# vivian556123/NeurIPS2024-CoVoMix

Hardware: AMD Instinct MI355X
Metric: mel-frames/sec (VoMix 32-step + HiFi-GAN, Bx1000x80) (higher is better)
Workload: dtype f16x3->f32 (fp32 operands split into fp16 hi/lo pairs, 3 MFMA products, fp32 accumulate); 1 GPU; VoMix 32-NFE (16 midpoint steps, CFG 0.7) + HiFi-GAN config_covomix, B=8 utterances x T=1000 frames per GPU, prompt 400; per_gpu_batch=8, frames=1000, nfe=32, parallelism=dp1 (utterance-sharded)

## Files before the change

include/covomix_hip.h:

```cpp
#ifndef COVOMIX_HIP_H
#define COVOMIX_HIP_H

#include <stdint.h>

#ifdef __cplusplus
extern "C" {
#endif

#define CVX_OK      0
#define CVX_EINVAL (-22)
#define CVX_EHIP   (-5)

#define CVX_ACT_NONE 0
#define CVX_ACT_GELU 1
#define CVX_ACT_SILU 2
#define CVX_ACT_TANH 3

typedef struct cvx_ctx {
    void*     stream;
    uint32_t* sat_flag;
    int32_t   n_cus;
    int32_t   flags;
} cvx_ctx;
#define CVX_CTX_NO_SATURATION_FLAG 1
typedef const cvx_ctx* cvx_stream_t;

#define CVX_ABI_VERSION 109
int         cvx_version(void);
const char* cvx_last_error_string(void);

int cvx_saturation_flag_reset(cvx_stream_t ctx);
int cvx_saturation_flag_query(uint32_t* host_out, int32_t reset, cvx_stream_t ctx);

int cvx_clock_stamps(uint64_t* stamps_dev, cvx_stream_t ctx);
int cvx_stream_create_cu_mask(const uint32_t* mask, int32_t n_words, void** out_stream);
int cvx_stream_destroy(void* stream);

typedef struct {
    const float* A;   int64_t lda;
    const float* A2;  int64_t lda2;  int32_t K1;
    const float* W;   int64_t ldw;
    float*       C;   int64_t ldc;
    const float* bias;
    const float* residual; int64_t ldr;
    int32_t M, N, K;
    int32_t act;
    const float* rope_cos; const float* rope_sin; int32_t rope_T; int32_t rope_cols;
} cvx_gemm_args;
int cvx_gemm_bias_act_f32(const cvx_gemm_args* a, cvx_stream_t s);

// ... 53 lines not shown
int cvx_attention_f16x3(const uint16_t* qk_hi, const uint16_t* qk_lo, const uint16_t* vt_hi, const uint16_t* vt_lo,
                        float* out, uint16_t* out_hi, uint16_t* out_lo,
                        int32_t Bt, int32_t T, int32_t Tp, int32_t H, float scale, cvx_stream_t s);
int cvx_attention_f16x3_scaled(const uint16_t* qk_hi, const uint16_t* qk_lo, const uint16_t* vt_hi, const uint16_t* vt_lo,
                               float* out, uint16_t* out_hi, uint16_t* out_lo,
                               int32_t Bt, int32_t T, int32_t Tp, int32_t H, float scale,
                               const float* qk_scale_dev, const float* v_scale_dev, const float* out_scale_dev, cvx_stream_t s);
int cvx_attention_f16x3_varlen(const uint16_t* qk_hi, const uint16_t* qk_lo, const uint16_t* vt_hi, const uint16_t* vt_lo,
                               float* out, uint16_t* out_hi, uint16_t* out_lo, const int32_t* cu_seqlens_dev,
                               int32_t n_seq, int32_t max_T, int64_t M, int32_t vt_ld, int32_t H, float scale,
                               const float* qk_scale_dev, const float* v_scale_dev, const float* out_scale_dev, cvx_stream_t s);

#define CVX_ATT_FORM_A 0
#define CVX_ATT_FORM_B 1
#define CVX_ATT_FORM_C 2
#define CVX_ATT_FORM_SINGLE_TERM 3
int cvx_attention_f16x3_form(int32_t n_seq, int32_t max_T, int64_t q_rows, int32_t H, int32_t single_term,
                             int32_t* query_block, int32_t* key_groups, int32_t* query_waves);

int cvx_dwconv31_gelu_res_f32(const float* x, const float* w, const float* bias, float* y,
                              int32_t Bt, int32_t T, int32_t C, cvx_stream_t s);
int cvx_dwconv31_gelu_res_varlen_f32(const float* x, const float* w, const float* bias, float* y,
                                     const int32_t* cu_seqlens_dev, int32_t n_seq, int32_t max_T, int32_t C, cvx_stream_t s);
int cvx_gemm_skinny_f32(const float* A, int32_t lda, const float* W, int64_t ldw, const float* bias, float* C, int64_t ldc,
                        int32_t M, int32_t N, int32_t K, int32_t act, cvx_stream_t s);
int cvx_cfg_combine_axpy_f32(const float* f_c, const float* f_n, const float* y, float cond_scale,
                             float coef, float* out, float* out2, float* out3, int64_t n, cvx_stream_t s);

int cvx_embed_gather_f32(const int64_t* ids, int32_t S, const float* table, int32_t E, int32_t n_rows_table,
                         const float* cond, const float* cond_row, int32_t Cc, int64_t null_id,
                         float* out, int64_t M, cvx_stream_t s);

int cvx_time_fourier_f32(const float* times, const float* w, float* out, int32_t n, int32_t half,
                         cvx_stream_t s);

typedef struct { const int32_t* item_len_dev; int32_t mul, add; } cvx_item_lengths;
typedef struct {
    const float* x;  int32_t B, Cin, Lin;
    const float* Wp; const float* bias;
    float* out;      int32_t Cout, Lout;
    int32_t ksize, dil, pad, up;
    float in_slope;
    const float* res; const float* accum; float out_scale;
    cvx_item_lengths items;
} cvx_conv_args;
int     cvx_hifigan_conv1d_f32(const cvx_conv_args* a, cvx_stream_t s);
// ... 188 lines not shown
```

neurips2024-covomix_amd/_lib.py:

```python
from __future__ import annotations

import ctypes as C
import os

import torch

_HERE = os.path.dirname(os.path.abspath(__file__))
LIB_PATH = os.environ.get("CVX_LIB_PATH") or os.path.join(_HERE, "libcovomix_hip.so")

_f32p = C.POINTER(C.c_float)
ABI_VERSION = 109


class GemmArgs(C.Structure):
    _fields_ = [
        ("A", C.c_void_p), ("lda", C.c_int64),
        ("A2", C.c_void_p), ("lda2", C.c_int64), ("K1", C.c_int32),
        ("W", C.c_void_p), ("ldw", C.c_int64),
        ("C", C.c_void_p), ("ldc", C.c_int64),
        ("bias", C.c_void_p),
        ("residual", C.c_void_p), ("ldr", C.c_int64),
        ("M", C.c_int32), ("N", C.c_int32), ("K", C.c_int32),
        ("act", C.c_int32),
        ("rope_cos", C.c_void_p), ("rope_sin", C.c_void_p), ("rope_T", C.c_int32), ("rope_cols", C.c_int32),
    ]


class GemmSplitIO(C.Structure):
    _fields_ = [
        ("A_hi", C.c_void_p), ("A_lo", C.c_void_p), ("lda_h", C.c_int64),
        ("A2_hi", C.c_void_p), ("A2_lo", C.c_void_p), ("lda2_h", C.c_int64),
        ("C_hi", C.c_void_p), ("C_lo", C.c_void_p), ("ldc_h", C.c_int64),
        ("write_f32", C.c_int32),
        ("Vt_hi", C.c_void_p), ("Vt_lo", C.c_void_p), ("vt_ld", C.c_int64),
# ... 184 lines not shown
                                                      C.c_int32, C.c_int32, C.c_int32, C.c_float, C.c_void_p, C.c_void_p]),
    "cvx_amax_pow2_scale_f32": (C.c_int, [C.c_void_p, C.c_int64, C.c_float, C.c_void_p, C.c_void_p, C.c_void_p]),
    "cvx_split_f16_dev": (C.c_int, [C.c_void_p, C.c_void_p, C.c_void_p, C.c_int64, C.c_float, C.c_void_p, C.c_void_p]),
    "cvx_split_f16_colscale_il": (C.c_int, [C.c_void_p, C.c_int64, C.c_int32, C.c_int32, C.c_void_p, C.c_int64, C.c_void_p, C.c_int64, C.c_int32,
                                            C.c_float, C.c_void_p, C.c_void_p]),
    "cvx_rownorm_scale_f32": (C.c_int, [C.c_void_p, C.c_int64, C.c_int32, C.c_int64, C.c_float, C.c_float, C.c_void_p, C.c_void_p]),
    "cvx_adarmsnorm_scaled_f32": (C.c_int, [C.c_void_p, C.c_void_p, C.c_void_p, C.c_void_p, C.c_void_p, C.c_void_p, C.c_int64,
                                            C.c_int32, C.c_int64, C.c_float, C.c_float, C.c_void_p, C.c_void_p]),
    "cvx_attention_f16x3_scaled": (C.c_int, [C.c_void_p, C.c_void_p, C.c_void_p, C.c_void_p, C.c_void_p, C.c_void_p, C.c_void_p,
                                             C.c_int32, C.c_int32, C.c_int32, C.c_int32, C.c_float, C.c_void_p, C.c_void_p,
                                             C.c_void_p, C.c_void_p]),
    "cvx_gemm_f16x3": (C.c_int, [C.POINTER(GemmArgs), C.c_void_p, C.c_void_p, C.c_float, C.POINTER(GemmSplitIO),
                                 C.c_void_p]),
    "cvx_gemm_f16x3_norm": (C.c_int, [C.POINTER(GemmArgs), C.c_void_p, C.c_void_p, C.c_float, C.POINTER(GemmSplitIO),
                                      C.POINTER(GemmNorm), C.c_void_p]),
    "cvx_adarmsnorm_f32": (C.c_int, [C.c_void_p, C.c_void_p, C.c_void_p, C.c_void_p, C.c_void_p, C.c_void_p, C.c_int64, C.c_int32,
                                     C.c_int64, C.c_float, C.c_float, C.c_void_p]),
    "cvx_attention_f32": (C.c_int, [C.c_void_p, C.c_void_p, C.c_void_p, C.c_void_p, C.c_int32, C.c_int32, C.c_int32, C.c_float,
                                    C.c_void_p]),
    "cvx_attention_f16x3": (C.c_int, [C.c_void_p, C.c_void_p, C.c_void_p, C.c_void_p, C.c_void_p, C.c_void_p, C.c_void_p,
                                      C.c_int32, C.c_int32, C.c_int32, C.c_int32, C.c_float, C.c_void_p]),
    "cvx_dwconv31_gelu_res_f32": (C.c_int, [C.c_void_p, C.c_void_p, C.c_void_p, C.c_void_p, C.c_int32, C.c_int32,
                                            C.c_int32, C.c_void_p]),
    "cvx_cfg_combine_axpy_f32": (C.c_int, [C.c_void_p, C.c_void_p, C.c_void_p, C.c_float, C.c_float, C.c_void_p,
                                           C.c_void_p, C.c_void_p, C.c_int64, C.c_void_p]),
    "cvx_embed_gather_f32": (C.c_int, [C.c_void_p, C.c_int32, C.c_void_p, C.c_int32, C.c_int32, C.c_void_p,
                                       C.c_void_p, C.c_int32, C.c_int64, C.c_void_p, C.c_int64, C.c_void_p]),
    "cvx_time_fourier_f32": (C.c_int, [C.c_void_p, C.c_void_p, C.c_void_p, C.c_int32, C.c_int32, C.c_void_p]),
    "cvx_hifigan_conv1d_f32": (C.c_int, [C.POINTER(ConvArgs), C.c_void_p]),
    "cvx_hifigan_packed_weight_floats": (C.c_int64, [C.c_int32, C.c_int32, C.c_int32]),
    "cvx_hifigan_pack_weight_f32": (C.c_int, [C.c_void_p, C.c_int32, C.c_int32, C.c_int32, C.c_int32, C.c_void_p]),
    "cvx_hifigan_post_f32": (C.c_int, [C.c_void_p, C.c_void_p, C.c_float, C.c_void_p, C.c_int32, C.c_int32,
                                       C.c_int32, C.c_float, C.c_void_p]),
    "cvx_wav_to_int16": (C.c_int, [C.c_void_p, C.c_void_p, C.c_int64, C.c_void_p]),
    "cvx_saturation_flag_reset": (C.c_int, [C.c_void_p]),
    "cvx_saturation_flag_query": (C.c_int, [C.POINTER(C.c_uint32), C.c_int32, C.c_void_p]),
    "cvx_stream_create_cu_mask": (C.c_int, [C.POINTER(C.c_uint32), C.c_int32, C.POINTER(C.c_void_p)]),
    "cvx_stream_destroy": (C.c_int, [C.c_void_p]),
    "cvx_clock_stamps": (C.c_int, [C.c_void_p, C.c_void_p]),
    "cvx_attention_varlen_f32": (C.c_int, [C.c_void_p, C.c_void_p, C.c_void_p, C.c_void_p, C.c_void_p, C.c_int32, C.c_int32,
                                           C.c_int32, C.c_float, C.c_void_p]),
    "cvx_attention_f16x3_varlen": (C.c_int, [C.c_void_p, C.c_void_p, C.c_void_p, C.c_void_p, C.c_void_p, C.c_void_p, C.c_void_p,
                                             C.c_void_p, C.c_int32, C.c_int32, C.c_int64, C.c_int32, C.c_int32, C.c_float,
                                             C.c_void_p, C.c_void_p, C.c_void_p, C.c_void_p]),
    "cvx_attention_f16x3_form": (C.c_int, [C.c_int32, C.c_int32, C.c_int64, C.c_int32, C.c_int32, C.POINTER(C.c_int32), C.POINTER(C.c_int32),
                                           C.POINTER(C.c_int32)]),
# ... 48 lines not shown
```

neurips2024-covomix_amd/acoustic.py:

```python
from __future__ import annotations

from typing import Dict, List, Optional

import os

import torch

from . import ops


def _dims_from_state(sd: Dict[str, torch.Tensor]) -> dict:
    dim, e_in = sd["to_embed.weight"].shape
    dim_cond = sd["null_cond"].shape[0]
    dim_emb = sd["to_phoneme_emb.weight"].shape[1]
    depth = 0
    while f"transformer.layers.{depth}.2.to_qkv.weight" in sd:
        depth += 1
    inner = sd["transformer.layers.0.2.to_qkv.weight"].shape[0] // 3
    dim_out = sd["to_pred.weight"].shape[0]
    streams = (e_in - dim_out - dim_cond) // dim_emb
    if dim_out + streams * dim_emb + dim_cond != e_in or inner % 64 != 0:
        raise ValueError("unsupported CoVoMix checkpoint geometry")
    return dict(dim=dim, e_in=e_in, dim_cond=dim_cond, dim_emb=dim_emb, depth=depth, heads=inner // 64,
                dim_head=64, dim_out=dim_out, streams=streams,
# ... 290 lines not shown
                and self.d["dim"] % 64 == 0 and 512 <= self.d["dim"] <= 4096 and os.environ.get("CVX_DEFER_NORM", "1") == "1"):
            return False
        return True

    def _deferred_norm_tables(self, table: torch.Tensor, HS: torch.Tensor, times_key) -> dict:
        d, sd = self.d, self.sd
        n, L, dim = table.shape[0], d["depth"], d["dim"]
        tab = table.view(n, L, 4, dim)
        tiny = torch.finfo(torch.float32).tiny
        gmax = tab[:, :, 0::2, :].abs().amax(dim=-1)
        gs = torch.exp2(-torch.ceil(torch.log2(gmax.clamp_min(tiny))).clamp(-40, 40)).contiguous()
        AS = (gs * HS[None, :, 1:3]).contiguous()

        def beta_w(beta_rows: torch.Tensor, w: torch.Tensor, bias) -> torch.Tensor:
            out = torch.empty(n, w.shape[0], dtype=torch.float32, device=self.device)
            for r0 in range(0, n, 32):
                r1 = min(n, r0 + 32)
                ops.gemm_skinny(beta_rows[r0:r1], w, out[r0:r1], bias=bias)
            return out
        key = (n, L, times_key)
        bufs = self._dn_bufs.get(key)
        if bufs is None:
            mk = lambda N: torch.empty(n, N, 2 * dim, dtype=torch.float16, device=self.device)
            bufs = dict(wq=[None if i == 0 else mk(3 * d["heads"] * 64) for i in range(L)], w1=[mk(4 * dim) for _ in range(L)])
            self._dn_bufs[key] = bufs
        b1p, bq, wq, w1 = [], [], [], []
        for i in range(L):
            p = f"transformer.layers.{i}"
            nq, n1 = p + ".2.to_qkv.weight", p + ".4.0.weight"
            b1p.append(beta_w(tab[:, i, 3, :], sd[n1], sd[p + ".4.0.bias"]))
            inv1 = self.split_il[n1][1]
            ops.split_f16_colscale_il(sd[n1], tab[:, i, 2, :], gs[:, i, 1], 1.0 / inv1, bufs["w1"][i])
            w1.append([(bufs["w1"][i][e], inv1) for e in range(n)])
            if i == 0:
                bq.append(None); wq.append(None)
                continue
            bq.append(beta_w(tab[:, i, 1, :], sd[nq], None))
            invq = self.split_il[nq][1]
            ops.split_f16_colscale_il(sd[nq], tab[:, i, 0, :], gs[:, i, 0], 1.0 / invq, bufs["wq"][i])
            wq.append([(bufs["wq"][i][e], invq) for e in range(n)])
        a0, h0 = AS.data_ptr(), HS.data_ptr()
        return dict(b1p=b1p, bq=bq, wq=wq, w1=w1, gs=gs, AS=AS, HS=HS, hsp=[[h0 + 4 * (4 * i + k) for k in range(4)] for i in range(L)],
                         asp=[[(a0 + 4 * ((e * L + i) * 2), a0 + 4 * ((e * L + i) * 2 + 1)) for i in range(L)] for e in range(n)])

    def _layers_pair_stream(self, ctx: dict, step: int, ws: dict, h: torch.Tensor, twin: dict, free: list, Bt: int, T: int, M: int, rg):
        d, sd, dn = self.d, self.sd, ctx["dn"]
        dim, L = d["dim"], d["depth"]
        tab = ctx["table"][step]
        sp, il = self.split.get, self.split_il.get
        sp_step, pp, hsp = ctx["sp"][step], self.pred_scale.data_ptr(), dn["hsp"]
        cur = hsp[0][0]
        take = free.pop
        parts64, rt_dim = dim // 64, float(dim) ** 0.5
        n16, a16, f16 = ws["normed16"], ws["att16"], ws["ff16"]
        rowsq = ws["rowsq"]
        rs = ws["rs"]
        def factor():
            ops.rownorm_scale(rowsq, M, parts64, rs, rt_dim)
        fkw = dict(a_row_scale=rs)
        skips: List[tuple] = []
        have_rs = False
        for i in range(L):
            p = f"transformer.layers.{i}"
            s_na, s_qk, s_v, s_at, s_nf, s_ff = sp_step[i]
            as_a, as_f = dn["asp"][step][i]
            last = i + 1 == L
            if self.has_comb[i]:
                s, s_scale = skips.pop()
                comb = take()
                ops.gemm(h, sd[p + ".0.weight"], comb, bias=sd[p + ".0.bias"], a2=s, w_split=sp(p + ".0.weight"), w_il=il(p + ".0.weight"),
                         a_split=twin[id(h)], a2_split=twin[id(s)], a_scale=cur, a2_scale=s_scale, out_split=twin[id(comb)], c_scale=hsp[i][1],
                         c_rowsq=rowsq, write_f32=False)
                cur = hsp[i][1]
                factor()
                have_rs = True
                free += [h, s]
                h, keep_input = comb, False
            else:
                skips.append((h, cur))
                keep_input = True
            nq = p + ".2.to_qkv.weight"
            if have_rs:
                ops.gemm(ws["normed"], sd[nq], ws["qkv"], rope=ws["rope"], rope_cols=2 * d["heads"] * 64, w_split=sp(nq), w_il=dn["wq"][i][step],
                         a_split=twin[id(h)], out_split=ws["qk16"], vt_split=ws["vt16"], write_f32=False, a_scale=as_a, c_scale=s_qk, vt_scale=s_v,
                         bias=dn["bq"][i][step], **fkw)
            else:
                ops.adarmsnorm(h, tab[(4 * i) * dim:(4 * i + 1) * dim], tab[(4 * i + 1) * dim:(4 * i + 2) * dim], None, out_split=n16, split_scale=s_na)
                ops.gemm(ws["normed"], sd[nq], ws["qkv"], rope=ws["rope"], rope_cols=2 * d["heads"] * 64, w_split=sp(nq), w_il=il(nq),
                         a_split=n16, out_split=ws["qk16"], vt_split=ws["vt16"], write_f32=False, a_scale=s_na, c_scale=s_qk, vt_scale=s_v)
            ops.attention_f16x3(ws["qk16"], ws["vt16"], None, Bt, T, d["heads"], 64 ** -0.5, out_split=a16,
                                qk_scale=s_qk, v_scale=s_v, out_scale=s_at, ragged=rg)
            h_att = take() if keep_input else h
            no = p + ".2.to_out.weight"
            ops.gemm(ws["att"], sd[no], h_att, w_split=sp(no), w_il=il(no), a_split=a16, a_scale=s_at, res_split=twin[id(h)], res_scale=cur,
                     out_split=twin[id(h_att)], c_scale=hsp[i][2], c_rowsq=rowsq, write_f32=False)
            cur = hsp[i][2]
            factor()
            h = h_att
            n1, n2 = p + ".4.0.weight", p + ".4.2.weight"
            ops.gemm(ws["normed"], sd[n1], ws["ff"], bias=dn["b1p"][i][step], act=ops.ACT_GELU, w_split=sp(n1), w_il=dn["w1"][i][step],
                     a_split=twin[id(h)], out_split=f16, write_f32=False, a_scale=as_f, c_scale=s_ff, **fkw)
            next_defers = (not last) and not self.has_comb[i + 1]
            ops.gemm(ws["ff"], sd[n2], h, bias=sd[p + ".4.2.bias"], w_split=sp(n2), w_il=il(n2), a_split=f16, a_scale=s_ff,
                     res_split=twin[id(h)], res_scale=cur, out_split=twin[id(h)], c_scale=hsp[i][3], c_rowsq=rowsq if next_defers else None,
                     write_f32=last)
            cur = hsp[i][3]
            if next_defers:
                factor()
            have_rs = next_defers
        ops.adarmsnorm(h, sd["transformer.final_norm.gamma"], None, None, out_split=ws["pred16"], split_scale=pp)
        ops.gemm(ws["normed"], sd["to_pred.weight"], ws["pred"], w_split=sp("to_pred.weight"), a_split=ws["pred16"], a_scale=pp,
                 w_il=il("to_pred.weight") if isinstance(ws["pred16"], ops.SplitIL) else None)
        return ws["pred"]

    @staticmethod
    def _ws_cut(ws: dict, r0: int, r1: int, vt) -> dict:

        def cut(v, lo=r0, hi=r1):
            if isinstance(v, ops.SplitIL):
                return v.rows_view(lo, hi)
            if isinstance(v, tuple):
                return tuple(None if t is None else t[lo:hi] for t in v)
            if isinstance(v, list):
                return [cut(t, lo, hi) for t in v]
            return v[lo:hi]
        out = {}
        for k, v in ws.items():
            if k == "rope":
                out[k] = v
            elif k == "vt16":
                out[k] = v if vt is None else cut(v, vt[0], vt[1])
            else:
                out[k] = cut(v)
        return out

    def evaluate(self, ctx: dict, step: int) -> torch.Tensor:
        d, sd, ws = self.d, self.sd, ctx["ws"]
        Bt, T, M, rg = ctx["Bt"], ctx["T"], ctx["M"], ctx.get("ragged")
        dim = d["dim"]
        tab = ctx["table"][step]
        free: List[torch.Tensor] = list(ws["h"])
        take = free.pop
        il = self.split_il.get
        if self.precision == "f16":
            split_io = M > 64 and dim % 64 == 0
            sp = self.split.get if split_io else (lambda k: None)
        else:
            split_io = self.precision == "f16x3" and M > 64 and dim % 32 == 0
            sp = self.split.get

        h = take()
        h0 = take()
        ops.gemm(ws["xin"], sd["to_embed.weight"][:, : d["dim_out"]], h0, residual=ws["base"])
        ops.dwconv31_gelu_res(h0, self.dw_w, sd["conv_embed.dw_conv1d.0.bias"], h, Bt, T, ragged=rg)
        free.append(h0)
        twin = {id(b): pr for b, pr in zip(ws["h"], ws["h16"])} if split_io else None
        sp_step = ctx["sp"][step] if (split_io and "sp" in ctx) else None
        hp = ctx["hp"] if sp_step is not None else None
        pp = self.pred_scale.data_ptr() if sp_step is not None else None
        use_dn = split_io and M >= 2048 and ctx.get("dn") is not None
        if split_io:
            tw = twin[id(h)]
            h0s = ctx["dn"]["hsp"][0][0] if use_dn else hp
            ops.split_act_f16(h, tw, scale=h0s) if isinstance(tw, ops.SplitIL) else ops.split_act_f16(h, *tw, scale=h0s)

        fuse_norm = split_io and M < 2048
        normed_ahead = False
        if use_dn:
            return self._layers_pair_stream(ctx, step, ws, h, twin, free, Bt, T, M, rg)
        def tab_rows(i_, k_):
            return tab[(4 * i_ + k_) * dim:(4 * i_ + k_ + 1) * dim]
        skips: List[torch.Tensor] = []
        for i in range(d["depth"]):
            p = f"transformer.layers.{i}"
            g_attn = tab[(4 * i + 0) * dim:(4 * i + 1) * dim]
            b_attn = tab[(4 * i + 1) * dim:(4 * i + 2) * dim]
            g_ff = tab[(4 * i + 2) * dim:(4 * i + 3) * dim]
            b_ff = tab[(4 * i + 3) * dim:(4 * i + 4) * dim]
            if (p + ".0.weight") in sd:
                s = skips.pop()
                comb = take()
                if split_io:
                    nm = dict(gamma=g_attn, beta=b_attn, out_split=ws["normed16"],
                              scale=sp_step[i][0] if sp_step is not None else None) if fuse_norm else None
                    ops.gemm(h, sd[p + ".0.weight"], comb, bias=sd[p + ".0.bias"], a2=s, w_split=sp(p + ".0.weight"), w_il=il(p + ".0.weight"),
                             a_split=twin[id(h)], a2_split=twin[id(s)], a_scale=hp, norm=nm)
                    normed_ahead = nm is not None
                else:
                    ops.gemm(h, sd[p + ".0.weight"], comb, bias=sd[p + ".0.bias"], a2=s, w_split=sp(p + ".0.weight"))
                free += [h, s]
                h, keep_input = comb, False
            else:
# ... 186 lines not shown
```

neurips2024-covomix_amd/csrc/elementwise.hip:

```cpp
#include "cvx_common.h"
#include <algorithm>
#include <stdarg.h>
#include <string.h>

static thread_local char g_err[512] = "";
void cvx_set_error(const char* fmt, ...)
{
    va_list ap;
    va_start(ap, fmt);
    vsnprintf(g_err, sizeof(g_err), fmt, ap);
    va_end(ap);
}
extern "C" const char* cvx_last_error_string(void) { return g_err; }

#include <mutex>
#include <map>
#include <set>
#include <utility>
void cvx_allow_dynamic_lds(const void* kernel, int bytes)
{
    static std::mutex mu;
    static std::map<std::pair<int, const void*>, int> granted;
    int dev = 0;
    if (hipGetDevice(&dev) != hipSuccess) dev = 0;
// ... 179 lines not shown
        const f32x4 t = *reinterpret_cast<const f32x4*>(xr + 4 * j);
        ss += t[0] * t[0] + t[1] * t[1] + t[2] * t[2] + t[3] * t[3];
    }
    ss = wave_sum(ss);
    const float inv = scale / fmaxf(sqrtf(ss), eps);
    for (int j = lane; j < (D >> 2); j += 64) {
        const f32x4 t = *reinterpret_cast<const f32x4*>(xr + 4 * j);
        const f32x4 gg = *reinterpret_cast<const f32x4*>(gamma + g * D + 4 * j);
        f32x4 o;
#pragma unroll
        for (int e = 0; e < 4; ++e) o[e] = t[e] * inv * gg[e];
        if (beta) {
            const f32x4 bb = *reinterpret_cast<const f32x4*>(beta + g * D + 4 * j);
#pragma unroll
            for (int e = 0; e < 4; ++e) o[e] += bb[e];
        }
        if (y) *reinterpret_cast<f32x4*>(y + row * D + 4 * j) = o;
        if (y_hi) { const f32x4 os = {o[0] * ssc, o[1] * ssc, o[2] * ssc, o[3] * ssc}; store_split4(y_hi, y_lo, row * D + 4 * j, os, amax); }
    }
    cvx_sat_commit(sat, amax);
}

constexpr int DW_K = 31, DW_TT = 16;
__global__ __launch_bounds__(256) void dwconv31_kernel(const float* __restrict__ x, const float* __restrict__ w,
                                                      const float* __restrict__ bias, float* __restrict__ y,
                                                      int T, int C, const int* __restrict__ cu_seqlens)
{
    const int c = blockIdx.x * 256 + threadIdx.x;
    if (c >= C) return;
    const int t0 = blockIdx.y * DW_TT;
    int64_t base = (int64_t)blockIdx.z * T * C;
    if (cu_seqlens) {
        const int r0 = cu_seqlens[blockIdx.z];
        T = cu_seqlens[blockIdx.z + 1] - r0;
        base = (int64_t)r0 * C;
        if (t0 >= T) return;
    }
    float wk[DW_K];
#pragma unroll
    for (int k = 0; k < DW_K; ++k) wk[k] = w[c * DW_K + k];
    float xs[DW_TT + DW_K - 1];
#pragma unroll
    for (int i = 0; i < DW_TT + DW_K - 1; ++i) {
        const int t = t0 + i - DW_K / 2;
        xs[i] = (t >= 0 && t < T) ? x[base + (int64_t)t * C + c] : 0.f;
    }
    const float bc = bias[c];
#pragma unroll
    for (int o = 0; o < DW_TT; o += 2) {
        float a0 = bc, a1 = bc;
#pragma unroll
        for (int k = 0; k < DW_K; ++k) { a0 = fmaf(wk[k], xs[o + k], a0); a1 = fmaf(wk[k], xs[o + 1 + k], a1); }
        const f32x2 g2 = gelu_fast2(f32x2{a0, a1});
        const int t = t0 + o;
        if (t < T) y[base + (int64_t)t * C + c] = g2[0] + xs[o + DW_K / 2];
        if (t + 1 < T) y[base + (int64_t)(t + 1) * C + c] = g2[1] + xs[o + 1 + DW_K / 2];
    }
}

constexpr int SK_M = 32;
constexpr int SK_KC = 1024;
constexpr int SK_Q = 16;
__global__ __launch_bounds__(256) void gemm_skinny_kernel(const float* __restrict__ A, int lda, const float* __restrict__ W, int64_t ldw,
                                                         const float* __restrict__ bias, float* __restrict__ Cm, int64_t ldc,
                                                         int M, int N, int K, int act)
{
    extern __shared__ __attribute__((aligned(16))) float sk_a[];
    const int tid = threadIdx.x, lane = tid & 63, wid = tid >> 6;
    const int KC = min(K, SK_KC), ldA = KC + 4;
    const int i31 = lane & 31, g = lane >> 5;
    const float* ar = sk_a + (size_t)i31 * ldA + 4 * g;
    const int n_tiles = (N + 31) / 32;
    for (int tile0 = blockIdx.x * 4; tile0 < n_tiles; tile0 += gridDim.x * 4) {
        const int tile = tile0 + wid;
        const bool active = tile < n_tiles;
        const int n0 = tile * 32;
        f32x16 acc0, acc1;
#pragma unroll
        for (int r = 0; r < 16; ++r) { acc0[r] = 0.f; acc1[r] = 0.f; }
        for (int kc = 0; kc < K; kc += KC) {
// ... 263 lines not shown
    if (hipMemsetAsync(scratch_dev, 0, sizeof(uint32_t), st) != hipSuccess) { cvx_set_error("amax_pow2_scale: memset failed"); return CVX_EHIP; }
    CVX_CHECK_LAUNCH("cvx_amax_pow2_scale_f32");
    return CVX_OK;
}

extern "C" int cvx_pow2_scale_from_amax_f32(uint32_t* amax_bits_dev, float target, float* scale_dev, cvx_stream_t s)
{
    CVX_REQUIRE(amax_bits_dev && scale_dev && target > 0.f, "pow2_scale_from_amax: bad arguments");
    hipStream_t st = cvx_hip_stream(s);
    hipLaunchKernelGGL(pow2_scale_kernel, dim3(1), dim3(1), 0, st, amax_bits_dev, target, scale_dev);
    if (hipMemsetAsync(amax_bits_dev, 0, sizeof(uint32_t), st) != hipSuccess) { cvx_set_error("pow2_scale_from_amax: memset failed"); return CVX_EHIP; }
    CVX_CHECK_LAUNCH("cvx_pow2_scale_from_amax_f32");
    return CVX_OK;
}

extern "C" int cvx_dwconv31_gelu_res_varlen_f32(const float* x, const float* w, const float* bias, float* y,
                                                const int32_t* cu_seqlens_dev, int32_t Bt, int32_t max_T, int32_t C, cvx_stream_t s)
{
    CVX_REQUIRE(x && w && bias && y, "dwconv31: null pointer");
    CVX_REQUIRE(Bt >= 0 && max_T > 0 && C > 0 && Bt <= 65535, "dwconv31: bad shape");
    CVX_REQUIRE(x != y, "dwconv31: in-place operation is not supported");
    if (Bt == 0) return CVX_OK;
    dim3 grid((C + 255) / 256, (max_T + DW_TT - 1) / DW_TT, Bt);
    hipLaunchKernelGGL(dwconv31_kernel, grid, dim3(256), 0, cvx_hip_stream(s), x, w, bias, y, max_T, C, cu_seqlens_dev);
    CVX_CHECK_LAUNCH("cvx_dwconv31_gelu_res_f32");
    return CVX_OK;
}

extern "C" int cvx_gemm_skinny_f32(const float* A, int32_t lda, const float* W, int64_t ldw, const float* bias, float* C, int64_t ldc,
                                   int32_t M, int32_t N, int32_t K, int32_t act, cvx_stream_t s)
{
    CVX_REQUIRE(A && W && C && M >= 0 && M <= SK_M && N >= 0 && K > 0 && K % 8 == 0 && lda >= K && lda % 4 == 0 && ldw >= K &&
                ldw % 4 == 0 && ldc >= N && act >= CVX_ACT_NONE && act <= CVX_ACT_TANH,
                "gemm_skinny: M <= 32, K a multiple of 8, lda / ldw multiples of 4 (M=%d N=%d K=%d)", M, N, K);
    CVX_REQUIRE(((uintptr_t)A & 15) == 0 && ((uintptr_t)W & 15) == 0, "gemm_skinny: 16-byte aligned operands");
    if (M == 0 || N == 0) return CVX_OK;
    const size_t lds = (size_t)SK_M * (std::min(K, SK_KC) + 4) * sizeof(float);
    cvx_allow_dynamic_lds(reinterpret_cast<const void*>(&gemm_skinny_kernel), (int)lds);
    const int64_t groups = ((int64_t)N + 127) / 128;
    const unsigned grid = (unsigned)std::min<int64_t>(groups, (int64_t)cvx_ctx_cus(s));
    hipLaunchKernelGGL(gemm_skinny_kernel, dim3(grid), dim3(256), lds, cvx_hip_stream(s), A, lda, W, ldw, bias, C, ldc, M, N, K, act);
    CVX_CHECK_LAUNCH("cvx_gemm_skinny_f32");
    return CVX_OK;
}

extern "C" int cvx_dwconv31_gelu_res_f32(const float* x, const float* w, const float* bias, float* y,
                                         int32_t Bt, int32_t T, int32_t C, cvx_stream_t s)
{
// ... 45 lines not shown
```

neurips2024-covomix_amd/csrc/gemm_f32.hip:

```cpp
#include "gemm_common.h"
#include <stdlib.h>

namespace {

using namespace cvxg;
constexpr int LDS_LD = BK + 4;

template <int TM>
__device__ __forceinline__ void mfma_group(const float* a, const float* b, int q, f32x16 (&acc)[TM][2])
{
    f32x4 af[TM], bf[2];
#pragma unroll
    for (int mi = 0; mi < TM; ++mi) af[mi] = *reinterpret_cast<const f32x4*>(a + mi * 32 * LDS_LD + q * 8);
#pragma unroll
    for (int ni = 0; ni < 2; ++ni) bf[ni] = *reinterpret_cast<const f32x4*>(b + ni * 32 * LDS_LD + q * 8);
#pragma unroll
    for (int t = 0; t < 4; ++t)
#pragma unroll
        for (int mi = 0; mi < TM; ++mi)
#pragma unroll
            for (int ni = 0; ni < 2; ++ni)
                acc[mi][ni] = __builtin_amdgcn_mfma_f32_32x32x2f32(af[mi][t], bf[ni][t], acc[mi][ni], 0, 0, 0);
}

// ... 253 lines not shown
#pragma unroll
    for (int mi = 0; mi < TM; ++mi)
#pragma unroll
        for (int ni = 0; ni < 2; ++ni)
#pragma unroll
            for (int r = 0; r < 16; ++r) acc[mi][ni][r] = 0.f;
    const int a_off = (wm * TM * 32 + (lane & 31)) * LDS_LD + (lane >> 5) * 4;
    const int b_off = (wn * 64 + (lane & 31)) * LDS_LD + (lane >> 5) * 4;
    const int nk = (p.K + BK - 1) / BK;
    load_tiles(0);
    store_tiles(0);
    __syncthreads();
    for (int kt = 0; kt < nk; ++kt) {
        const int cur = kt & 1;
        if (kt + 1 < nk) load_tiles((kt + 1) * BK);
        const float* a = As + cur * BM * LDS_LD + a_off;
        const float* b = Bs + cur * BN * LDS_LD + b_off;
#pragma unroll
        for (int q = 0; q < 4; ++q) mfma_group<TM>(a, b, q, acc);
        if (kt + 1 < nk) store_tiles(cur ^ 1);
        __syncthreads();
    }
    gemm_epilogue<TM>(p, acc, m0, n0, wm, wn, lane);
}

template <int TM>
int launch_gemm(const cvx_gemm_args& a, hipStream_t st)
{
    constexpr int BM = TM * 64;
    const size_t lds = (size_t)2 * (BM + BN) * LDS_LD * sizeof(float);
    const bool fast = (a.K % BK == 0);
    cvx_allow_dynamic_lds(fast ? reinterpret_cast<const void*>(gemm_f32_kernel<TM>)
                               : reinterpret_cast<const void*>(gemm_f32_generic_kernel<TM>), (int)lds);
    const int tiles_n = (a.N + BN - 1) / BN, tiles_m = (a.M + BM - 1) / BM;
    const int map_mode = 1;
    const int grid_m = map_mode == 1 ? ((tiles_m + 7) / 8) * 8 : tiles_m;
    dim3 grid((unsigned)(grid_m * tiles_n));
    if constexpr (TM == 2) {
        if (fast) {
            const size_t lds_dma = (size_t)4 * 128 * BK * sizeof(float);
            cvx_allow_dynamic_lds(reinterpret_cast<const void*>(gemm_f32_glds_kernel), (int)lds_dma);
            hipLaunchKernelGGL(gemm_f32_glds_kernel, grid, dim3(256), lds_dma, st, a, tiles_m, tiles_n, map_mode);
            CVX_CHECK_LAUNCH("cvx_gemm_bias_act_f32");
            return CVX_OK;
        }
    }
// ... 10 lines not shown
    CVX_REQUIRE(a != nullptr, "gemm: null args");
    CVX_REQUIRE(a->M >= 0 && a->N > 0 && a->K > 0, "gemm: bad shape M=%d N=%d K=%d", a->M, a->N, a->K);
    CVX_REQUIRE(a->A && a->W && a->C, "gemm: null operand");
    CVX_REQUIRE(a->K % 4 == 0 && a->lda % 4 == 0 && a->ldw % 4 == 0, "gemm: K/lda/ldw must be multiples of 4");
    CVX_REQUIRE((((uintptr_t)a->A | (uintptr_t)a->W) & 15) == 0, "gemm: A/W must be 16-byte aligned");
    if (a->A2) {
        CVX_REQUIRE(a->K1 > 0 && a->K1 < a->K && a->K1 % BK == 0 && a->lda2 % 4 == 0 &&
                    (((uintptr_t)a->A2) & 15) == 0, "gemm: bad split-K operand (K1=%d)", a->K1);
    }
    if (a->rope_cos) {
        CVX_REQUIRE(a->rope_sin && a->rope_T > 0 && a->rope_cols % 64 == 0 && a->rope_cols <= a->N,
                    "gemm: bad RoPE epilogue arguments");
    }
    CVX_REQUIRE(a->act >= CVX_ACT_NONE && a->act <= CVX_ACT_SILU, "gemm: unsupported activation %d", a->act);
    return CVX_OK;
}

extern "C" int cvx_gemm_bias_act_f32(const cvx_gemm_args* a, cvx_stream_t s)
{
    const int rc = cvxg::validate_gemm_args(a);
    if (rc != CVX_OK) return rc;
    if (a->M == 0) return CVX_OK;
    hipStream_t st = cvx_hip_stream(s);
    const long blocks128 = (long)((a->M + 127) / 128) * ((a->N + BN - 1) / BN);
    if (a->M <= 64 || blocks128 < 256) return launch_gemm<1>(*a, st);
    return launch_gemm<2>(*a, st);
}
```

neurips2024-covomix_amd/ops.py:

```python
from __future__ import annotations

import ctypes as C
import os as _os
import functools
import threading
from contextlib import contextmanager
from typing import Optional

import torch

from . import _lib
from ._lib import ConvArgs, GemmArgs, GemmNorm, GemmSplitIO

ACT_NONE, ACT_GELU, ACT_SILU = 0, 1, 2


_CTX: dict = {}


def ctx_of(stream: Optional["torch.cuda.Stream"] = None) -> "_lib.Ctx":
    st = stream if stream is not None else torch.cuda.current_stream()
    key = (st.device.index, st.cuda_stream)
    c = _CTX.get(key)
    if c is None:
# ... 623 lines not shown
def geglu(h: torch.Tensor, out: torch.Tensor, F: int) -> torch.Tensor:
    _chk_f32(h, out)
    assert h.is_contiguous() and out.is_contiguous() and h.shape[-1] == 2 * F and out.shape[-1] >= F and h.shape[0] == out.shape[0]
    _lib.check(_lib.load().cvx_geglu_f32(h.data_ptr(), out.data_ptr(), h.shape[0], F, out.shape[-1], _stream()), "cvx_geglu_f32")
    return out


def dwconv31_gelu_res(x: torch.Tensor, w: torch.Tensor, bias: torch.Tensor, out: torch.Tensor,
                      Bt: int, T: int, ragged: Optional[Ragged] = None) -> torch.Tensor:
    _chk_f32(x, w, bias, out)
    C_ = x.shape[-1]
    assert x.is_contiguous() and out.is_contiguous() and w.is_contiguous() and w.numel() == C_ * 31
    if ragged is not None:
        assert x.numel() == ragged.M * C_
        _lib.check(_lib.load().cvx_dwconv31_gelu_res_varlen_f32(x.data_ptr(), w.data_ptr(), bias.data_ptr(), out.data_ptr(),
                                                                ragged.cu.data_ptr(), ragged.n, ragged.max_T, C_, _stream()),
                   "cvx_dwconv31_gelu_res_varlen_f32")
        return out
    _lib.check(_lib.load().cvx_dwconv31_gelu_res_f32(x.data_ptr(), w.data_ptr(), bias.data_ptr(), out.data_ptr(),
                                                     Bt, T, C_, _stream()), "cvx_dwconv31_gelu_res_f32")
    return out


def gemm_skinny(a: torch.Tensor, w: torch.Tensor, out: torch.Tensor, *, bias=None, act: int = ACT_NONE) -> torch.Tensor:
    _chk_f32(a, w, out, bias)
    M, K = a.shape
    N = w.shape[0]
    assert w.shape[1] == K and tuple(out.shape) == (M, N) and a.stride(1) == 1 and w.stride(1) == 1 and out.stride(1) == 1
    _lib.check(_lib.load().cvx_gemm_skinny_f32(a.data_ptr(), a.stride(0), w.data_ptr(), w.stride(0), _p(bias), out.data_ptr(), out.stride(0),
                                               M, N, K, act, _stream()), "cvx_gemm_skinny_f32")
    return out


def cfg_combine_axpy(f_c, f_n, y, cond_scale: float, coef: float, out, out2=None, out3=None) -> None:
    _chk_f32(f_c, f_n, y, out, out2, out3)
    n = y.numel()
    assert f_c.numel() == n and out.numel() == n and (f_n is None or f_n.numel() == n)
    for t in (f_c, f_n, y, out, out2, out3):
        assert t is None or t.is_contiguous()
    _lib.check(_lib.load().cvx_cfg_combine_axpy_f32(f_c.data_ptr(), _p(f_n), y.data_ptr(), cond_scale, coef,
                                                    out.data_ptr(), _p(out2), _p(out3), n, _stream()),
               "cvx_cfg_combine_axpy_f32")


def embed_gather(ids: Optional[torch.Tensor], streams: int, table: torch.Tensor, cond: Optional[torch.Tensor],
                 cond_row: Optional[torch.Tensor], cond_dim: int, null_id: int, out: torch.Tensor, M: int) -> torch.Tensor:
# ... 380 lines not shown
```

Before: 22020 mel-frames/s.

## Fuse dwconv embed with fp16 split and row norms; stream K=80 embed GEMM

The depthwise conv+GELU+residual kernel can now write the fp16 hi/lo split of the hidden state directly, along with per-row squared sums, and then compute the row-norm factor. This lets layer 0 skip its separate split pass and adaptive RMSNorm and use the pre-folded qkv weights like the other layers. A dedicated streaming MFMA kernel for the K=80 input embedding GEMM with residual is also added; it keeps weights in registers and prefetches row tiles. The trade-off is more template code, a per-element wave reduction inside the conv loop, and folded layer-0 weight buffers that must be prepared per step.

```diff
diff --git a/include/covomix_hip.h b/include/covomix_hip.h
--- a/include/covomix_hip.h
+++ b/include/covomix_hip.h
@@ -25,7 +25,7 @@
 #define CVX_CTX_NO_SATURATION_FLAG 1
 typedef const cvx_ctx* cvx_stream_t;
 
-#define CVX_ABI_VERSION 109
+#define CVX_ABI_VERSION 110
 int         cvx_version(void);
 const char* cvx_last_error_string(void);
 
@@ -125,6 +125,10 @@
                               int32_t Bt, int32_t T, int32_t C, cvx_stream_t s);
 int cvx_dwconv31_gelu_res_varlen_f32(const float* x, const float* w, const float* bias, float* y,
                                      const int32_t* cu_seqlens_dev, int32_t n_seq, int32_t max_T, int32_t C, cvx_stream_t s);
+int cvx_dwconv31_gelu_res_split(const float* x, const float* w, const float* bias, uint16_t* y_hi, uint16_t* y_lo, int64_t ldy_h,
+                                const float* scale_dev, float* rowsq, int64_t rowsq_ld, float* row_factor, float factor_scale,
+                                float factor_eps, const int32_t* cu_seqlens_dev, int32_t Bt, int32_t T, int32_t C, int64_t rows,
+                                cvx_stream_t s);
 int cvx_gemm_skinny_f32(const float* A, int32_t lda, const float* W, int64_t ldw, const float* bias, float* C, int64_t ldc,
                         int32_t M, int32_t N, int32_t K, int32_t act, cvx_stream_t s);
 int cvx_cfg_combine_axpy_f32(const float* f_c, const float* f_n, const float* y, float cond_scale,
diff --git a/neurips2024-covomix_amd/_lib.py b/neurips2024-covomix_amd/_lib.py
--- a/neurips2024-covomix_amd/_lib.py
+++ b/neurips2024-covomix_amd/_lib.py
@@ -9,7 +9,7 @@
 LIB_PATH = os.environ.get("CVX_LIB_PATH") or os.path.join(_HERE, "libcovomix_hip.so")
 
 _f32p = C.POINTER(C.c_float)
-ABI_VERSION = 109
+ABI_VERSION = 110
 
 
 class GemmArgs(C.Structure):
@@ -240,6 +240,9 @@
                                       C.c_int32, C.c_int32, C.c_int32, C.c_int32, C.c_float, C.c_void_p]),
     "cvx_dwconv31_gelu_res_f32": (C.c_int, [C.c_void_p, C.c_void_p, C.c_void_p, C.c_void_p, C.c_int32, C.c_int32,
                                             C.c_int32, C.c_void_p]),
+    "cvx_dwconv31_gelu_res_split": (C.c_int, [C.c_void_p, C.c_void_p, C.c_void_p, C.c_void_p, C.c_void_p, C.c_int64, C.c_void_p, C.c_void_p,
+                                              C.c_int64, C.c_void_p, C.c_float, C.c_float, C.c_void_p, C.c_int32, C.c_int32, C.c_int32,
+                                              C.c_int64, C.c_void_p]),
     "cvx_cfg_combine_axpy_f32": (C.c_int, [C.c_void_p, C.c_void_p, C.c_void_p, C.c_float, C.c_float, C.c_void_p,
                                            C.c_void_p, C.c_void_p, C.c_int64, C.c_void_p]),
     "cvx_embed_gather_f32": (C.c_int, [C.c_void_p, C.c_int32, C.c_void_p, C.c_int32, C.c_int32, C.c_void_p,
diff --git a/neurips2024-covomix_amd/acoustic.py b/neurips2024-covomix_amd/acoustic.py
--- a/neurips2024-covomix_amd/acoustic.py
+++ b/neurips2024-covomix_amd/acoustic.py
@@ -336,7 +336,7 @@
         bufs = self._dn_bufs.get(key)
         if bufs is None:
             mk = lambda N: torch.empty(n, N, 2 * dim, dtype=torch.float16, device=self.device)
-            bufs = dict(wq=[None if i == 0 else mk(3 * d["heads"] * 64) for i in range(L)], w1=[mk(4 * dim) for _ in range(L)])
+            bufs = dict(wq=[mk(3 * d["heads"] * 64) for _ in range(L)], w1=[mk(4 * dim) for _ in range(L)])
             self._dn_bufs[key] = bufs
         b1p, bq, wq, w1 = [], [], [], []
         for i in range(L):
@@ -346,9 +346,6 @@
             inv1 = self.split_il[n1][1]
             ops.split_f16_colscale_il(sd[n1], tab[:, i, 2, :], gs[:, i, 1], 1.0 / inv1, bufs["w1"][i])
             w1.append([(bufs["w1"][i][e], inv1) for e in range(n)])
-            if i == 0:
-                bq.append(None); wq.append(None)
-                continue
             bq.append(beta_w(tab[:, i, 1, :], sd[nq], None))
             invq = self.split_il[nq][1]
             ops.split_f16_colscale_il(sd[nq], tab[:, i, 0, :], gs[:, i, 0], 1.0 / invq, bufs["wq"][i])
@@ -360,20 +357,18 @@
     def _layers_pair_stream(self, ctx: dict, step: int, ws: dict, h: torch.Tensor, twin: dict, free: list, Bt: int, T: int, M: int, rg):
         d, sd, dn = self.d, self.sd, ctx["dn"]
         dim, L = d["dim"], d["depth"]
-        tab = ctx["table"][step]
         sp, il = self.split.get, self.split_il.get
         sp_step, pp, hsp = ctx["sp"][step], self.pred_scale.data_ptr(), dn["hsp"]
         cur = hsp[0][0]
         take = free.pop
         parts64, rt_dim = dim // 64, float(dim) ** 0.5
-        n16, a16, f16 = ws["normed16"], ws["att16"], ws["ff16"]
+        a16, f16 = ws["att16"], ws["ff16"]
         rowsq = ws["rowsq"]
         rs = ws["rs"]
         def factor():
             ops.rownorm_scale(rowsq, M, parts64, rs, rt_dim)
         fkw = dict(a_row_scale=rs)
         skips: List[tuple] = []
-        have_rs = False
         for i in range(L):
             p = f"transformer.layers.{i}"
             s_na, s_qk, s_v, s_at, s_nf, s_ff = sp_step[i]
@@ -387,21 +382,15 @@
                          c_rowsq=rowsq, write_f32=False)
                 cur = hsp[i][1]
                 factor()
-                have_rs = True
                 free += [h, s]
                 h, keep_input = comb, False
             else:
                 skips.append((h, cur))
                 keep_input = True
             nq = p + ".2.to_qkv.weight"
-            if have_rs:
-                ops.gemm(ws["normed"], sd[nq], ws["qkv"], rope=ws["rope"], rope_cols=2 * d["heads"] * 64, w_split=sp(nq), w_il=dn["wq"][i][step],
-                         a_split=twin[id(h)], out_split=ws["qk16"], vt_split=ws["vt16"], write_f32=False, a_scale=as_a, c_scale=s_qk, vt_scale=s_v,
-                         bias=dn["bq"][i][step], **fkw)
-            else:
-                ops.adarmsnorm(h, tab[(4 * i) * dim:(4 * i + 1) * dim], tab[(4 * i + 1) * dim:(4 * i + 2) * dim], None, out_split=n16, split_scale=s_na)
-                ops.gemm(ws["normed"], sd[nq], ws["qkv"], rope=ws["rope"], rope_cols=2 * d["heads"] * 64, w_split=sp(nq), w_il=il(nq),
-                         a_split=n16, out_split=ws["qk16"], vt_split=ws["vt16"], write_f32=False, a_scale=s_na, c_scale=s_qk, vt_scale=s_v)
+            ops.gemm(ws["normed"], sd[nq], ws["qkv"], rope=ws["rope"], rope_cols=2 * d["heads"] * 64, w_split=sp(nq), w_il=dn["wq"][i][step],
+                     a_split=twin[id(h)], out_split=ws["qk16"], vt_split=ws["vt16"], write_f32=False, a_scale=as_a, c_scale=s_qk, vt_scale=s_v,
+                     bias=dn["bq"][i][step], **fkw)
             ops.attention_f16x3(ws["qk16"], ws["vt16"], None, Bt, T, d["heads"], 64 ** -0.5, out_split=a16,
                                 qk_scale=s_qk, v_scale=s_v, out_scale=s_at, ragged=rg)
             h_att = take() if keep_input else h
@@ -421,7 +410,6 @@
             cur = hsp[i][3]
             if next_defers:
                 factor()
-            have_rs = next_defers
         ops.adarmsnorm(h, sd["transformer.final_norm.gamma"], None, None, out_split=ws["pred16"], split_scale=pp)
         ops.gemm(ws["normed"], sd["to_pred.weight"], ws["pred"], w_split=sp("to_pred.weight"), a_split=ws["pred16"], a_scale=pp,
                  w_il=il("to_pred.weight") if isinstance(ws["pred16"], ops.SplitIL) else None)
@@ -466,22 +454,24 @@
         h = take()
         h0 = take()
         ops.gemm(ws["xin"], sd["to_embed.weight"][:, : d["dim_out"]], h0, residual=ws["base"])
-        ops.dwconv31_gelu_res(h0, self.dw_w, sd["conv_embed.dw_conv1d.0.bias"], h, Bt, T, ragged=rg)
-        free.append(h0)
         twin = {id(b): pr for b, pr in zip(ws["h"], ws["h16"])} if split_io else None
         sp_step = ctx["sp"][step] if (split_io and "sp" in ctx) else None
         hp = ctx["hp"] if sp_step is not None else None
         pp = self.pred_scale.data_ptr() if sp_step is not None else None
         use_dn = split_io and M >= 2048 and ctx.get("dn") is not None
+        if use_dn:
+            ops.dwconv31_gelu_res_split(h0, self.dw_w, sd["conv_embed.dw_conv1d.0.bias"], twin[id(h)], Bt, T, scale=ctx["dn"]["hsp"][0][0],
+                                        rowsq=ws["rowsq"], row_factor=ws["rs"], factor_scale=float(dim) ** 0.5, ragged=rg)
+            free.append(h0)
+            return self._layers_pair_stream(ctx, step, ws, h, twin, free, Bt, T, M, rg)
+        ops.dwconv31_gelu_res(h0, self.dw_w, sd["conv_embed.dw_conv1d.0.bias"], h, Bt, T, ragged=rg)
+        free.append(h0)
         if split_io:
             tw = twin[id(h)]
-            h0s = ctx["dn"]["hsp"][0][0] if use_dn else hp
-            ops.split_act_f16(h, tw, scale=h0s) if isinstance(tw, ops.SplitIL) else ops.split_act_f16(h, *tw, scale=h0s)
+            ops.split_act_f16(h, tw, scale=hp) if isinstance(tw, ops.SplitIL) else ops.split_act_f16(h, *tw, scale=hp)
 
         fuse_norm = split_io and M < 2048
         normed_ahead = False
-        if use_dn:
-            return self._layers_pair_stream(ctx, step, ws, h, twin, free, Bt, T, M, rg)
         def tab_rows(i_, k_):
             return tab[(4 * i_ + k_) * dim:(4 * i_ + k_ + 1) * dim]
         skips: List[torch.Tensor] = []
diff --git a/neurips2024-covomix_amd/csrc/elementwise.hip b/neurips2024-covomix_amd/csrc/elementwise.hip
--- a/neurips2024-covomix_amd/csrc/elementwise.hip
+++ b/neurips2024-covomix_amd/csrc/elementwise.hip
@@ -225,9 +225,11 @@
 }
 
 constexpr int DW_K = 31, DW_TT = 16;
+struct DwSplit { _Float16* hi; _Float16* lo; int64_t ld; const float* scale; float* rowsq; int64_t rowsq_ld; uint32_t* sat; };
+template <bool SPLIT>
 __global__ __launch_bounds__(256) void dwconv31_kernel(const float* __restrict__ x, const float* __restrict__ w,
                                                       const float* __restrict__ bias, float* __restrict__ y,
-                                                      int T, int C, const int* __restrict__ cu_seqlens)
+                                                      int T, int C, const int* __restrict__ cu_seqlens, const DwSplit sp)
 {
     const int c = blockIdx.x * 256 + threadIdx.x;
     if (c >= C) return;
@@ -249,6 +251,10 @@
         xs[i] = (t >= 0 && t < T) ? x[base + (int64_t)t * C + c] : 0.f;
     }
     const float bc = bias[c];
+    CvxSat amax;
+    const int64_t row0 = base / C;
+    const float ssc = (SPLIT && sp.scale) ? *sp.scale : 1.f, inv_ssc = 1.f / ssc;
+    const bool il = SPLIT && sp.lo == sp.hi + 32;
 #pragma unroll
     for (int o = 0; o < DW_TT; o += 2) {
         float a0 = bc, a1 = bc;
@@ -256,9 +262,31 @@
         for (int k = 0; k < DW_K; ++k) { a0 = fmaf(wk[k], xs[o + k], a0); a1 = fmaf(wk[k], xs[o + 1 + k], a1); }
         const f32x2 g2 = gelu_fast2(f32x2{a0, a1});
         const int t = t0 + o;
-        if (t < T) y[base + (int64_t)t * C + c] = g2[0] + xs[o + DW_K / 2];
-        if (t + 1 < T) y[base + (int64_t)(t + 1) * C + c] = g2[1] + xs[o + 1 + DW_K / 2];
-    }
+        const float y0 = g2[0] + xs[o + DW_K / 2], y1 = g2[1] + xs[o + 1 + DW_K / 2];
+        if constexpr (!SPLIT) {
+            if (t < T) y[base + (int64_t)t * C + c] = y0;
+            if (t + 1 < T) y[base + (int64_t)(t + 1) * C + c] = y1;
+        } else {
+            const float yv[2] = {y0, y1};
+#pragma unroll
+            for (int e = 0; e < 2; ++e) {
+                if (t + e >= T) break;
+                const int64_t row = row0 + t + e;
+                const float v = yv[e] * ssc;
+                cvx_amax3(amax, v, v);
+                const float xc = fminf(fmaxf(v, -65504.f), 65504.f);
+                const _Float16 h = (_Float16)xc;
+                const _Float16 l = (_Float16)(xc - (float)h);
+                const int64_t off = row * sp.ld + (il ? (((c >> 5) << 6) | (c & 31)) : c);
+                sp.hi[off] = h;
+                if (sp.lo) sp.lo[off] = l;
+                const float r = ((float)h + (sp.lo ? (float)l : 0.f)) * inv_ssc;
+                const float q = wave_sum(r * r);
+                if (sp.rowsq && (threadIdx.x & 63) == 0) sp.rowsq[row * sp.rowsq_ld + (c >> 6)] = q;
+            }
+        }
+    }
+    if constexpr (SPLIT) cvx_sat_commit(sp.sat, amax);
 }
 
 constexpr int SK_M = 32;
@@ -568,8 +596,29 @@
     CVX_REQUIRE(x != y, "dwconv31: in-place operation is not supported");
     if (Bt == 0) return CVX_OK;
     dim3 grid((C + 255) / 256, (max_T + DW_TT - 1) / DW_TT, Bt);
-    hipLaunchKernelGGL(dwconv31_kernel, grid, dim3(256), 0, cvx_hip_stream(s), x, w, bias, y, max_T, C, cu_seqlens_dev);
+    hipLaunchKernelGGL(dwconv31_kernel<false>, grid, dim3(256), 0, cvx_hip_stream(s), x, w, bias, y, max_T, C, cu_seqlens_dev, DwSplit{});
     CVX_CHECK_LAUNCH("cvx_dwconv31_gelu_res_f32");
+    return CVX_OK;
+}
+
+extern "C" int cvx_dwconv31_gelu_res_split(const float* x, const float* w, const float* bias, uint16_t* y_hi, uint16_t* y_lo, int64_t ldy_h,
+                                           const float* scale_dev, float* rowsq, int64_t rowsq_ld, float* row_factor, float factor_scale,
+                                           float factor_eps, const int32_t* cu_seqlens_dev, int32_t Bt, int32_t max_T, int32_t C,
+                                           int64_t rows, cvx_stream_t s)
+{
+    CVX_REQUIRE(x && w && bias && y_hi, "dwconv31_split: null pointer");
+    CVX_REQUIRE(Bt >= 0 && max_T > 0 && C > 0 && C % 64 == 0 && Bt <= 65535, "dwconv31_split: bad shape (C=%d: whole waves of 64 channels)", C);
+    CVX_REQUIRE(ldy_h >= (y_lo == y_hi + 32 ? 2 * (int64_t)C : (int64_t)C) && (!rowsq || rowsq_ld >= C / 64),
+                "dwconv31_split: bad strides (ldy_h=%ld rowsq_ld=%ld)", (long)ldy_h, (long)rowsq_ld);
+    CVX_REQUIRE(!row_factor || (rowsq && rows >= 0 && (cu_seqlens_dev || rows == (int64_t)Bt * max_T)),
+                "dwconv31_split: row_factor needs rowsq and the row count (rows=%ld)", (long)rows);
+    if (Bt == 0) return CVX_OK;
+    CVX_REQUIRE_SAT(s);
+    dim3 grid((C + 255) / 256, (max_T + DW_TT - 1) / DW_TT, Bt);
+    const DwSplit sp{reinterpret_cast<_Float16*>(y_hi), reinterpret_cast<_Float16*>(y_lo), ldy_h, scale_dev, rowsq, rowsq_ld, cvx_sat_flag_for(s)};
+    hipLaunchKernelGGL(dwconv31_kernel<true>, grid, dim3(256), 0, cvx_hip_stream(s), x, w, bias, (float*)nullptr, max_T, C, cu_seqlens_dev, sp);
+    CVX_CHECK_LAUNCH("cvx_dwconv31_gelu_res_split");
+    if (row_factor) return cvx_rownorm_scale_f32(rowsq, rows, C / 64, rowsq_ld, factor_scale, factor_eps, row_factor, s);
     return CVX_OK;
 }
 
diff --git a/neurips2024-covomix_amd/csrc/gemm_f32.hip b/neurips2024-covomix_amd/csrc/gemm_f32.hip
--- a/neurips2024-covomix_amd/csrc/gemm_f32.hip
+++ b/neurips2024-covomix_amd/csrc/gemm_f32.hip
@@ -299,6 +299,74 @@
         __syncthreads();
     }
     gemm_epilogue<TM>(p, acc, m0, n0, wm, wn, lane);
+}
+
+constexpr int STREAM_ROWS = 128;
+template <int KQ>
+__global__ __launch_bounds__(256, 2) void gemm_f32_stream_kernel(const cvx_gemm_args p)
+{
+    const int lane = threadIdx.x & 63, wid = threadIdx.x >> 6;
+    const int i31 = lane & 31, half = lane >> 5, qd = lane & 3;
+    const int colw = ((int)blockIdx.x * 4 + wid) * 64;
+    if (colw >= p.N) return;
+    f32x4 wb[2][KQ];
+#pragma unroll
+    for (int ni = 0; ni < 2; ++ni)
+#pragma unroll
+        for (int q = 0; q < KQ; ++q) wb[ni][q] = gload4(p.W + (int64_t)(colw + 32 * ni + i31) * p.ldw + 8 * q + 4 * half);
+    const int r_begin = (int)blockIdx.y * STREAM_ROWS, r_end = min(p.M, r_begin + STREAM_ROWS);
+    const int c4 = colw + 4 * (i31 >> 2);
+    f32x4 xa[KQ], rb[4][2];
+    auto load_tile = [&](int m0) {
+        const float* xr = p.A + (int64_t)min(m0 + i31, p.M - 1) * p.lda + 4 * half;
+#pragma unroll
+        for (int q = 0; q < KQ; ++q) xa[q] = gload4(xr + 8 * q);
+#pragma unroll
+        for (int rg = 0; rg < 4; ++rg) {
+            const float* rp = p.residual + (int64_t)min(m0 + 8 * rg + 4 * half + qd, p.M - 1) * p.ldr + c4;
+            rb[rg][0] = gload4(rp);
+            rb[rg][1] = gload4(rp + 32);
+        }
+    };
+    load_tile(r_begin);
+    for (int m0 = r_begin; m0 < r_end; m0 += 32) {
+        f32x16 acc[2];
+#pragma unroll
+        for (int ni = 0; ni < 2; ++ni)
+#pragma unroll
+            for (int r = 0; r < 16; ++r) acc[ni][r] = 0.f;
+#pragma unroll
+        for (int q = 0; q < KQ; ++q)
+#pragma unroll
+            for (int t = 0; t < 4; ++t)
+#pragma unroll
+                for (int ni = 0; ni < 2; ++ni)
+                    acc[ni] = __builtin_amdgcn_mfma_f32_32x32x2f32(xa[q][t], wb[ni][q][t], acc[ni], 0, 0, 0);
+        f32x4 rc[4][2];
+#pragma unroll
+        for (int rg = 0; rg < 4; ++rg) { rc[rg][0] = rb[rg][0]; rc[rg][1] = rb[rg][1]; }
+        if (m0 + 32 < r_end) load_tile(m0 + 32);
+#pragma unroll
+        for (int rg = 0; rg < 4; ++rg) {
+            float lo[4], hi[4];
+#pragma unroll
+            for (int e = 0; e < 4; ++e) { lo[e] = acc[0][4 * rg + e]; hi[e] = acc[1][4 * rg + e]; }
+            quad_transpose(lo[0], lo[1], lo[2], lo[3], lane);
+            quad_transpose(hi[0], hi[1], hi[2], hi[3], lane);
+            const int row = m0 + 8 * rg + 4 * half + qd;
+            if (row >= p.M) continue;
+            float* cp = p.C + (int64_t)row * p.ldc + c4;
+            *reinterpret_cast<f32x4*>(cp) = f32x4{lo[0], lo[1], lo[2], lo[3]} + rc[rg][0];
+            *reinterpret_cast<f32x4*>(cp + 32) = f32x4{hi[0], hi[1], hi[2], hi[3]} + rc[rg][1];
+        }
+    }
+}
+
+constexpr int STREAM_MIN_ROWS = 8192;
+bool stream_form(const cvx_gemm_args& a)
+{
+    return a.K == 80 && a.M >= STREAM_MIN_ROWS && a.N % 64 == 0 && !a.A2 && !a.bias && !a.rope_cos && a.act == CVX_ACT_NONE &&
+           a.residual && a.residual != a.C && (((uintptr_t)a.residual | (uintptr_t)a.C) & 15) == 0 && (a.ldr & 3) == 0 && (a.ldc & 3) == 0;
 }
 
 template <int TM>
@@ -355,6 +423,12 @@
     if (rc != CVX_OK) return rc;
     if (a->M == 0) return CVX_OK;
     hipStream_t st = cvx_hip_stream(s);
+    if (stream_form(*a)) {
+        const dim3 grid((unsigned)((a->N + 255) / 256), (unsigned)((a->M + STREAM_ROWS - 1) / STREAM_ROWS));
+        hipLaunchKernelGGL(gemm_f32_stream_kernel<10>, grid, dim3(256), 0, st, *a);
+        CVX_CHECK_LAUNCH("cvx_gemm_bias_act_f32");
+        return CVX_OK;
+    }
     const long blocks128 = (long)((a->M + 127) / 128) * ((a->N + BN - 1) / BN);
     if (a->M <= 64 || blocks128 < 256) return launch_gemm<1>(*a, st);
     return launch_gemm<2>(*a, st);
diff --git a/neurips2024-covomix_amd/ops.py b/neurips2024-covomix_amd/ops.py
--- a/neurips2024-covomix_amd/ops.py
+++ b/neurips2024-covomix_amd/ops.py
@@ -669,6 +669,28 @@
     return out
 
 
+def dwconv31_gelu_res_split(x: torch.Tensor, w: torch.Tensor, bias: torch.Tensor, out_split, Bt: int, T: int, *, scale=None,
+                            rowsq: Optional[torch.Tensor] = None, row_factor: Optional[torch.Tensor] = None, factor_scale: float = 1.0,
+                            eps: float = 1e-12, ragged: Optional[Ragged] = None):
+    _chk_f32(x, w, bias, rowsq, row_factor)
+    C_ = x.shape[-1]
+    rows = x.numel() // C_
+    assert x.is_contiguous() and w.is_contiguous() and w.numel() == C_ * 31 and C_ % 64 == 0
+    assert rows == (ragged.M if ragged is not None else Bt * T)
+    ensure_saturation_bound()
+    hi, lo, ld = _pair(out_split, rows if isinstance(out_split, SplitIL) else None, C_)
+    assert isinstance(out_split, SplitIL) or (out_split[0].ndim == 2 and out_split[0].shape[0] == rows)
+    if rowsq is not None:
+        assert rowsq.ndim == 2 and rowsq.shape[0] >= rows and rowsq.stride(1) == 1 and rowsq.shape[1] * 64 >= C_
+    cu, n, mt = (ragged.cu.data_ptr(), ragged.n, ragged.max_T) if ragged is not None else (None, Bt, T)
+    assert row_factor is None or (rowsq is not None and row_factor.numel() >= rows and row_factor.stride(-1) == 1)
+    _lib.check(_lib.load().cvx_dwconv31_gelu_res_split(x.data_ptr(), w.data_ptr(), bias.data_ptr(), hi, lo, ld, _sp(scale), _p(rowsq),
+                                                       rowsq.stride(0) if rowsq is not None else 0, _p(row_factor), factor_scale, eps,
+                                                       cu, n, mt, C_, rows, _stream()),
+               "cvx_dwconv31_gelu_res_split")
+    return out_split
+
+
 def gemm_skinny(a: torch.Tensor, w: torch.Tensor, out: torch.Tensor, *, bias=None, act: int = ACT_NONE) -> torch.Tensor:
     _chk_f32(a, w, out, bias)
     M, K = a.shape
```

Measured after the change: 22090 mel-frames/s (median of 6 runs). About the same (+0.3%).
